# channable/alfred-margaret

Hardware: AMD Instinct MI355X
Metric: GiB/s haystack bytes scanned (match-emitting runLower, 100k-needle automaton) (higher is better)
Workload: dtype u8

## Files before the change

### alfred-margaret_amd/api.py

```python
import ctypes as C
import os

import numpy as np

from . import build as _build

CASE_SENSITIVE = 0
IGNORE_CASE = 1

AM_OK = 0
AM_ERR_INVALID, AM_ERR_NO_DEVICE, AM_ERR_HIP, AM_ERR_OOM, AM_ERR_UNSUPPORTED = -1, -2, -3, -4, -5


class AmError(RuntimeError):
    def __init__(self, code, msg):
        super().__init__("libam error %d: %s" % (code, msg))
        self.code = code


class Slice(C.Structure):
    _fields_ = [("ptr", C.c_void_p), ("off", C.c_size_t), ("len", C.c_size_t)]


MATCH_DTYPE = np.dtype([("end_pos", np.uint64), ("haystack", np.uint32), ("state", np.uint32)])
# ... 947 lines not shown

def sf_unit_chunks(total_bytes, n_cu=0):
    uc = int(libam().am_debug_sf_unit_chunks(int(total_bytes), int(n_cu)))
    if uc == 0:
        raise AmError(AM_ERR_NO_DEVICE, (libam().am_last_error() or b"").decode("utf-8", "replace"))
    return uc


SF_MODES = ("count", "emit", "any", "ids")


def decode_sf_variant(word):
    word = int(word)
    if not word & 1:
        return None
    return {"ic": bool(word & 2), "mode": SF_MODES[(word >> 2) & 3], "ilp": (word >> 4) & 3, "lw": (word >> 16) & 255, "short": bool(word & 64), "dbg": bool(word & 128),
            "light": bool(word & 256), "children": bool(word & 512)}


def sf_last_variant():
    return decode_sf_variant(libam().am_debug_sf_last_variant())


def bounds_report():
    f, l, u = C.c_uint64(0), C.c_uint32(0), C.c_uint32(0)
    check(libam().am_debug_bounds_report(C.byref(f), C.byref(l), C.byref(u)))
    return int(f.value), int(l.value), int(u.value)


def image_version():
    return int(libam().am_image_version())


def lower_code_point(cp):
    return int(libam().am_lower_code_point(cp))


def unlower_code_point(cp):
    buf = (C.c_uint32 * 16)()
    n = libam().am_unlower_code_point(cp, buf, 16)
    return [int(buf[i]) for i in range(n)]


def lower_utf8(text):
    b = _as_bytes(text)
    out = C.create_string_buffer(len(b) * 4 + 4)
# ... 41 lines not shown
```

### alfred-margaret_amd/csrc/am_abi.cpp

```cpp
#include "am_host.h"

#include <condition_variable>
#include <deque>
#include <sys/mman.h>

using namespace am;
using namespace am::dev;
using namespace am::host;

static_assert(sizeof(am_match) == sizeof(Record), "am_match must mirror the device record");
static_assert(offsetof(am_match, end_pos) == offsetof(Record, end_pos) && offsetof(am_match, haystack) == offsetof(Record, haystack) &&
                  offsetof(am_match, state) == offsetof(Record, state), "am_match layout");


static thread_local std::string g_err;
namespace am { int abi_fail(int code, const std::string& msg) { g_err = msg; return code; } }

namespace am {
namespace host {

Runtime g_rt;

int ensure_runtime()
{
// ... 107 lines not shown
    }
    HIP_TRY(hipMemcpyAsync(tl_state.pin_res + off, d_src, n, hipMemcpyDeviceToHost, st));
    items[n_items++] = Item{dst, off, n};
    used = off + n;
    return AM_OK;
}
int am::host::ResultCopies::finish(hipStream_t st)
{
    HIP_TRY(hipStreamSynchronize(st));
    for (int i = 0; i < n_items; i++) std::memcpy(items[i].dst, tl_state.pin_res + items[i].off, items[i].n);
    return AM_OK;
}

namespace {
struct RecordCache {
    struct Block { void* p; size_t cap; };
    std::mutex mu; std::vector<Block> kept;
    void* take(size_t need, size_t* cap_out)
    {
        std::lock_guard<std::mutex> lk(mu);
        size_t best = kept.size();
        for (size_t i = 0; i < kept.size(); i++)
            if (kept[i].cap >= need && kept[i].cap <= 2 * need + (1u << 20) && (best == kept.size() || kept[i].cap < kept[best].cap)) best = i;
        if (best == kept.size()) return nullptr;
        void* r = kept[best].p; *cap_out = kept[best].cap;
        kept.erase(kept.begin() + (std::ptrdiff_t)best);
        return r;
    }
    void trim()
    {
        std::vector<Block> out;
        { std::lock_guard<std::mutex> lk(mu); out.swap(kept); }
        for (const Block& b : out) (void)hipFree(b.p);
    }
    void give(void* q, size_t c)
    {
        std::vector<Block> out;
        {
            std::lock_guard<std::mutex> lk(mu);
            kept.push_back(Block{q, c});
            size_t total = 0;
            for (const Block& b : kept) total += b.cap;
            while (kept.size() > 4 || (kept.size() > 1 && total > ((size_t)16 << 30))) { total -= kept.front().cap; out.push_back(kept.front()); kept.erase(kept.begin()); }
        }
        for (const Block& b : out) (void)hipFree(b.p);
    }
// ... 423 lines not shown
    if (limit == 0) {
        size_t free_b = 0, total_b = 0;
        OnDevice od(dev);
        limit = (od.rc == AM_OK && hipMemGetInfo(&free_b, &total_b) == hipSuccess) ? std::max<size_t>(total_b / 16, (size_t)256 << 20) : (size_t)256 << 20;
        keep[dev].store(limit, std::memory_order_relaxed);
    }
    if (held > limit) { am_batch_destroy(b); b = nullptr; }
}
}

int am::host::upload_batch(const am_slice* hay, size_t n_hay, am_batch* b, bool oneshot) { return upload_slices(hay, n_hay, b, oneshot); }
am_batch* am::host::oneshot_batch(int dev) { return oneshot_get(dev); }
void am::host::oneshot_batch_trim(int dev) { oneshot_trim(dev); }
int am::host::record_array_get(int dev, size_t need, void** p, size_t* cap)
{
    *p = g_record_cache[dev].take(need, cap);
    if (*p) return AM_OK;
    *cap = need + need / 16;
    hipError_t e = hipMalloc(p, *cap);
    if (e != hipSuccess) { *p = nullptr; *cap = 0; return fail(e == hipErrorOutOfMemory ? AM_ERR_OOM : AM_ERR_HIP, std::string("hipMalloc(records): ") + hipGetErrorString(e)); }
    return AM_OK;
}
void am::host::record_array_put(int dev, void* p, size_t cap) { if (p) g_record_cache[dev].give(p, cap); }

extern "C" int am_batch_from_device(const void* d_bytes, const void* d_offsets, size_t n_hay, uint64_t total_bytes, am_batch** out)
{
    if (!out) return fail(AM_ERR_INVALID, "out is null");
    *out = nullptr;
    if (!d_offsets || (total_bytes && !d_bytes)) return fail(AM_ERR_INVALID, "null device pointers");
    int dev = 0;
    AM_TRY(device_of_pointer(total_bytes ? d_bytes : d_offsets, &dev));
    ON_DEVICE(dev);
    if (((uintptr_t)d_bytes & 15) != 0) return fail(AM_ERR_INVALID, "d_bytes must be 16-byte aligned");
    if (n_hay >= 0xFFFFFFFFull) return fail(AM_ERR_INVALID, "too many haystacks");
    uint64_t first = 1, last = 0;
    HIP_TRY(hipMemcpy(&first, d_offsets, 8, hipMemcpyDeviceToHost));
    HIP_TRY(hipMemcpy(&last, (const uint64_t*)d_offsets + n_hay, 8, hipMemcpyDeviceToHost));
    if (first != 0 || last != total_bytes) return fail(AM_ERR_INVALID, "d_offsets[0] must be 0 and d_offsets[n_hay] must equal total_bytes");
    am_batch* b = new am_batch();
    b->dev = dev;
    b->owns = false; b->d_text = const_cast<void*>(d_bytes); b->d_offsets = (uint64_t*)const_cast<void*>(d_offsets);
    b->total = total_bytes; b->n_hay = (uint32_t)n_hay;
    int rc = finish_batch(b);
    if (rc != AM_OK) { am_batch_destroy(b); return rc; }
    *out = b;
    return AM_OK;
// ... 655 lines not shown
```

### alfred-margaret_amd/csrc/am_device.h

```cpp
#pragma once
#include <hip/hip_runtime.h>

#include "am_image.h"

namespace am {
namespace dev {

constexpr int kModeCount = 0;
constexpr int kModeEmit = 1;
constexpr int kModeAny = 2;
constexpr int kModeIds = 3;

struct alignas(16) Record { uint64_t end_pos; uint32_t haystack; uint32_t state; };

struct ScanOut {
    uint32_t* unit_counts;
    const uint64_t* unit_offsets;
    Record* records;
    Record* pool;
    uint32_t* block_next;
    uint32_t* pool_ctrl;
    uint32_t* unit_first;
    uint32_t* unit_slots;
    uint32_t wq_iters;
// ... 2 lines not shown
    uint32_t unit_chunks;
    uint32_t* next_unit;
    uint64_t* hay_counts;
    uint64_t* total_values;
    uint8_t* flags;
    const uint64_t* ids_vals_off; const uint32_t* ids_vals; uint32_t* ids_bits; uint32_t* ids_missing; uint32_t ids_words, ids_n;
    uint32_t two_always;
    uint64_t* dbg;
};

constexpr uint32_t kPoolBlock = 64;
constexpr uint32_t kSfBlockGrant = 32;
inline uint64_t pool_grant_slack(int n_cu, uint64_t n_units, bool two_per_cu)
{
    uint64_t w = (uint64_t)n_cu * (two_per_cu ? 32u : 16u);
    const uint64_t need = (n_units + 15u) / 16u * 16u;
    if (w > need) w = need;
    return w * kSfBlockGrant;
}

hipError_t launch_hidx(const BatchView& b, uint32_t* hidx, uint64_t n_entries, hipStream_t st, uint32_t* z0 = nullptr, uint64_t n0 = 0, uint32_t* z1 = nullptr, uint64_t n1 = 0);
uint64_t sf_chunks(const BatchView& b);
uint32_t sf_unit_chunks(const BatchView& b, int n_cu);
hipError_t launch_permute(const ScanOut& o, const uint64_t* unit_offsets, Record* out, uint64_t n_units, hipStream_t st);
uint64_t ac_units(const AcView& a, const BatchView& b);
size_t sf_lds_bytes(const SfView& s);
hipError_t launch_sf(bool ic, int mode, const SfView& s, const BatchView& b, const ScanOut& o, int n_cu, hipStream_t st);
uint32_t take_sf_last_variant();
hipError_t launch_ac(bool ic, int mode, const AcView& a, const BatchView& b, const ScanOut& o, hipStream_t st);
uint64_t dfa_units(const DfaView& d, const BatchView& b);
bool dfa_usable(const DfaView& d);
struct DfaLaunch {
    int n_cu; uint32_t workgroups, per_cu;
    uint32_t lds_rows, hot_rows, lds_n1, lds_n2;
    uint32_t walk; bool place_wide;
};
DfaLaunch dfa_launch_shape(const DfaView& d, const BatchView& b, int n_cu);
hipError_t launch_dfa(int mode, const DfaView& d, const BatchView& b, const ScanOut& o, const DfaLaunch& s, hipStream_t st);
hipError_t launch_dfa_sample(const DfaView& d, const uint8_t* text, uint64_t total, uint32_t n_samples, uint32_t len, uint32_t* out, hipStream_t st);
bool dfa_tokens_ok(const DfaView& d);
uint64_t dfa_token_superblocks(uint64_t records, uint32_t n_waves , uint64_t n_units);
uint64_t dfa_superblock_bytes();
hipError_t launch_dfa_tokens(const DfaView& d, const BatchView& b, const ScanOut& o, const DfaLaunch& s, hipStream_t st);
hipError_t launch_dfa_place(const DfaView& d, const BatchView& b, const ScanOut& o, uint32_t n_super, const uint64_t* unit_offsets, const DfaLaunch& s, uint32_t n_ref_states, Record* out, hipStream_t st);
hipError_t read_sf_phase_cycles(uint64_t* out5);
hipError_t read_sf_wave_records(uint64_t* out, size_t n_waves);
hipError_t scan_temp_bytes(uint64_t n, size_t* bytes);
hipError_t launch_scan(void* temp, size_t temp_bytes, const uint32_t* counts, uint64_t* offsets, uint64_t n, hipStream_t st);


hipError_t launch_dense(bool ic, bool write, const AcView& a, const BatchView& b, const Record* sparse, const uint64_t* sparse_offsets, uint32_t unit_chunks,
                        uint64_t n_units, uint32_t* unit_totals, const uint64_t* out_offsets, Record* out, hipStream_t st);
hipError_t launch_records_reduce(const Record* recs, uint64_t n, const uint32_t* vlen, uint64_t* hay_counts, uint64_t* total, uint8_t* flags, hipStream_t st);
hipError_t launch_range_bounds(const Record* recs, uint64_t n, uint64_t x0, uint64_t x1, uint64_t* out2, hipStream_t st);
hipError_t launch_range_rebase(Record* recs, uint64_t n, uint64_t add, hipStream_t st);
hipError_t launch_hay_rebase(Record* recs, uint64_t n, uint32_t add, hipStream_t st);
hipError_t launch_spin(uint32_t workgroups, uint32_t threads, uint64_t cycles, uint32_t* out, hipStream_t st);

struct RpPayload { int64_t priority; uint32_t len_bytes; uint32_t len_code_points; uint64_t repl_off; uint32_t repl_len; uint32_t reserved; };
struct RpStateOne { int32_t priority; uint32_t payload; };
constexpr uint32_t kRpWalkList = 0xFFFFFFFFu;
struct RpTables { const uint64_t* vals_off; const uint32_t* vals; const RpPayload* payloads; const uint8_t* repl; int64_t min_priority; const RpStateOne* one; };
struct RpKept { uint64_t src_start, src_len, dst; };
constexpr uint32_t kRpActive = 0, kRpFinished = 1, kRpNothing = 2;
struct RpHay { uint64_t newlen; int64_t best; uint32_t status, nkept, payload, pad; };
struct RpFin { uint64_t off, len; uint32_t orig, status; };
struct RpRoute { uint64_t* len_next; uint64_t* len_fin; uint32_t* tiles; uint32_t* act; uint32_t* fin; };
struct RpRouted { const uint64_t* off_next; const uint64_t* off_fin; const uint64_t* tile_off; const uint64_t* act_idx; const uint64_t* fin_idx; };
constexpr uint64_t kRpTile = 16384;

hipError_t launch_rp_ranges(const Record* recs, uint64_t n_rec, uint64_t* rec_first, const RpRoute& route, uint32_t n_act, hipStream_t st);
// ... 129 lines not shown
```

### alfred-margaret_amd/csrc/am_host.h

```cpp
#pragma once
#include "../../include/am.h"
#include "../../include/am_debug.h"

#include <hip/hip_runtime.h>

#include <algorithm>
#include <atomic>
#include <chrono>
#include <cstdio>
#include <cstdlib>
#include <cstring>
#include <functional>
#include <future>
#include <map>
#include <memory>
#include <mutex>
#include <string>
#include <thread>
#include <vector>

#include "am_config.h"
#include "am_device.h"
#include "am_flatten.h"

// ... 108 lines not shown
    bool has_ref = false;
    std::shared_ptr<const am::LowerTable> lower;
    std::vector<uint8_t> cs_image;
    struct Flat { int rc = 0; std::string err; std::vector<uint8_t> img; };
    std::future<Flat> ic_pending;
    int kernel_pref = 0;
    std::mutex mu;
    am::host::Flavor fl[2];
};

struct am_batch {
    int dev = 0;
    void* d_text = nullptr; uint64_t* d_offsets = nullptr;
    bool owns = false;
    bool hidx_ready = false;
    uint64_t total = 0; uint32_t n_hay = 0;
    std::mutex mu;
    am::host::DevBuf text_buf, offs_buf;
    am::host::DevBuf combo;
    am::host::DevBuf hidx, unit_counts, unit_offsets, scan_tmp, small, hay_counts, flags, unit_first, pool, block_next;
    am::host::DevBuf sparse, dense_counts, dense_offsets, dense_out;
    uint64_t route_image = 0; bool route_dfa = false;
    uint32_t route_ends_per_kib = 0;
};

struct am_matches {
    int dev = 0;
    am::dev::Record* d_records = nullptr; uint64_t n = 0; size_t cap_bytes = 0;
    uint64_t first = 0;
    std::vector<am_match> host; bool fetched = false;
    am_match* big = nullptr; size_t big_cap = 0;
    bool big_pinned = false;
};

struct am_needle_ids {
    const am_automaton* a = nullptr;
    uint32_t n_needles = 0;
    uint64_t n_states = 0, n_values = 0;
    am::host::DevBuf vals_off, vals;
};

namespace am {
namespace host {

struct ResultCopies {
    struct Item { void* dst; size_t off, n; };
    Item items[4]; int n_items = 0; size_t used = 0;
    int add(void* dst, const void* d_src, size_t n, hipStream_t st);
    int finish(hipStream_t st);
};

int prepare(const am_automaton* ca, int case_mode, const Flavor** out);
int finish_batch(am_batch* b);
int run_batch_impl(const am_automaton* a, int case_mode, const am_batch* cb, am_matches** out, bool allow_small);
int scan_needle_ids(const am_automaton* a, int case_mode, am_batch* b, const uint64_t* d_vals_off, const uint32_t* d_vals, uint32_t n_needles,
                    uint32_t* d_bits, uint32_t words, uint32_t* d_missing, uint8_t* flags_out, bool* taken);
int run_records(const am_automaton* a, int case_mode, am_batch* b, const std::function<int(uint64_t, Record**)>& sink_final, uint64_t* n_out, bool have_lock = false);
int run_records_async(const am_automaton* a, int case_mode, am_batch* b, Record* d_out, const uint64_t** n_dev, hipStream_t st);
int upload_batch(const am_slice* hay, size_t n_hay, am_batch* b, bool oneshot);
am_batch* oneshot_batch(int dev);
void oneshot_batch_trim(int dev);
int record_array_get(int dev, size_t need, void** p, size_t* cap);
void record_array_put(int dev, void* p, size_t cap);
struct RecordArray {
    int dev; void* p = nullptr; size_t cap = 0;
    explicit RecordArray(int d) : dev(d) {}
    int ensure(size_t need)
    {
        if (need <= cap) return AM_OK;
        record_array_put(dev, p, cap); p = nullptr; cap = 0;
        return record_array_get(dev, need, &p, &cap);
    }
    ~RecordArray() { record_array_put(dev, p, cap); }
};
inline size_t padded_text(uint64_t total) { return (size_t)((total + 15) & ~15ull) + 16; }
template <class Buf>
auto records_into(Buf& d, uint64_t spare = 0)
{
    return [&d, spare](uint64_t n, Record** ptr) -> int { AM_TRY(d.ensure((n + spare) * sizeof(Record))); *ptr = (Record*)d.p; return AM_OK; };
}
inline constexpr RpRoute kNoRoute{nullptr, nullptr, nullptr, nullptr, nullptr};

}
}
```

### alfred-margaret_amd/csrc/am_kernels.hip

```cpp
#include <hip/hip_runtime.h>

#include <atomic>
#include <cstdlib>
#include <type_traits>

#include "am_bounds.h"
#include "am_config.h"
#include "am_device.h"
#include "am_wave.h"

AM_BOUNDS_TU("am_kernels.hip")

namespace am {
namespace dev {


__global__ void k_hidx(const uint64_t* __restrict__ offsets, uint32_t n_hay, uint64_t total, uint32_t* __restrict__ hidx, uint64_t n_entries,
                       uint32_t* __restrict__ z0, uint64_t n0, uint32_t* __restrict__ z1, uint64_t n1)
{
    const uint64_t k = (uint64_t)blockIdx.x * blockDim.x + threadIdx.x;
    const uint64_t stride = (uint64_t)gridDim.x * blockDim.x;
    for (uint64_t i = k; i < n0; i += stride) z0[i] = 0u;
    for (uint64_t i = k; i < n1; i += stride) z1[i] = 0u;
    if (k >= n_entries) return;
// ... 602 lines not shown
        for (int i = 0; i < 7; i++) atomicAdd(reinterpret_cast<unsigned long long*>(o.dbg + 16 + 2 * 8192 + i), (unsigned long long)dbg_iters[i]);
        atomicAdd(reinterpret_cast<unsigned long long*>(o.dbg + 11), (unsigned long long)n_cand);
        atomicAdd(reinterpret_cast<unsigned long long*>(o.dbg + 12), (unsigned long long)n_probes);
        atomicAdd(reinterpret_cast<unsigned long long*>(o.dbg + 13), (unsigned long long)n_defer);
        atomicAdd(reinterpret_cast<unsigned long long*>(o.dbg + 14), (unsigned long long)n_found);
        atomicMax(reinterpret_cast<unsigned long long*>(o.dbg + 15), (unsigned long long)(__builtin_amdgcn_s_memtime() - t_begin));
        const uint64_t gw = (uint64_t)blockIdx.x * kSfWaves + wave;
        if (gw < 8192) {
            uint32_t hw_id, xcc_id;
            asm volatile("s_getreg_b32 %0, hwreg(HW_REG_HW_ID)" : "=s"(hw_id));
            asm volatile("s_getreg_b32 %0, hwreg(HW_REG_XCC_ID)" : "=s"(xcc_id));
            o.dbg[16 + 2 * gw] = __builtin_amdgcn_s_memtime() - t_begin;
            o.dbg[17 + 2 * gw] = ((uint64_t)xcc_id << 32) | hw_id;
        }
    }

    if (MODE == kModeCount) {
        if (o.hay_counts) flush_count();
        nval = wave_sum_u64(nval);
        if (lane == 0 && nval) atomicAdd(reinterpret_cast<unsigned long long*>(o.total_values), (unsigned long long)nval);
    }
}

__global__ __launch_bounds__(256) void k_permute(ScanOut o, const uint64_t* __restrict__ unit_offsets, Record* __restrict__ out, uint64_t n_units)
{
    const uint64_t u = ((uint64_t)blockIdx.x * blockDim.x + threadIdx.x) >> 6;
    const uint32_t lane = threadIdx.x & 63u;
    if (u >= n_units) return;
    const uint32_t n = o.unit_slots[u];
    uint64_t at = unit_offsets[u];
    uint32_t blk = o.unit_first[u];
    const uint4* pool4 = reinterpret_cast<const uint4*>(o.pool);
    uint4* out4 = reinterpret_cast<uint4*>(out);
    for (uint32_t done = 0; done < n; done += kPoolBlock) {
        if (blk == kNone) break;
        uint4 r = make_uint4(0u, 0u, 0u, kNone);
        if (done + lane < n) r = pool4[(uint64_t)blk * kPoolBlock + lane];
        const uint64_t m = __ballot(r.w != kNone);
        if (r.w != kNone) out4[at + (uint32_t)__popcll(m & ((1ull << lane) - 1ull))] = r;
        at += (uint32_t)__popcll(m);
        blk = o.block_next[blk];
    }
}


hipError_t launch_hidx(const BatchView& b, uint32_t* hidx, uint64_t n_entries, hipStream_t st, uint32_t* z0, uint64_t n0, uint32_t* z1, uint64_t n1)
{
    const uint32_t blocks = (uint32_t)((n_entries + 255) / 256);
    hipLaunchKernelGGL(k_hidx, dim3(blocks), dim3(256), 0, st, b.offsets, b.n_hay, b.total, hidx, n_entries, z0, n0, z1, n1);
    return hipGetLastError();
}

uint64_t sf_chunks(const BatchView& b) { return (b.total + kSfChunk - 1) / kSfChunk; }

uint32_t sf_unit_chunks(const BatchView& b, int n_cu)
{
    const uint64_t n_chunks = sf_chunks(b), waves = (uint64_t)(n_cu > 0 ? n_cu : 1) * kSfWaves;
    const uint64_t per_wave = (n_chunks + waves - 1) / waves;
    const uint64_t k = (per_wave + kSfMaxUnitChunks - 1) / kSfMaxUnitChunks;
    if (k >= 4) return kSfMaxUnitChunks;
    const uint64_t uc = k <= 1 ? per_wave : (n_chunks + waves * k - 1) / (waves * k);
    return (uint32_t)(uc < 1 ? 1 : uc);
}

hipError_t launch_permute(const ScanOut& o, const uint64_t* unit_offsets, Record* out, uint64_t n_units, hipStream_t st)
{
    if (n_units == 0) return hipSuccess;
    const uint64_t blocks = (n_units * 64 + 255) / 256;
    hipLaunchKernelGGL(k_permute, dim3((uint32_t)blocks), dim3(256), 0, st, o, unit_offsets, out, n_units);
    return hipGetLastError();
}
uint64_t ac_units(const AcView& a, const BatchView& b) { return (b.total + a.chunk - 1) / a.chunk; }

static size_t sf_lds_bytes_w(const SfView& s, int waves) { return kSfMaskBytes + ((size_t)4 << s.bloom_log2_words) + (size_t)waves * (kSfStage + kSfQ1 * sizeof(uint16_t) + kSfQ2 * sizeof(uint16_t)); }
static uint32_t sf_wq_cap(const SfView& s, int waves)
{
    const size_t base = sf_lds_bytes_w(s, waves), limit = 160 * 1024;
    if (base >= limit) return 0;
    size_t cap = (limit - base) / ((size_t)waves * 64);
    if (cap > 128) cap = 128;
    return cap >= 64 ? (uint32_t)cap : 0u;
}
size_t sf_lds_bytes(const SfView& s) { return sf_lds_bytes_w(s, kSfWaves); }

constexpr uint32_t kSfVariantValid = 1u, kSfVariantIc = 2u, kSfVariantModeShift = 2, kSfVariantIlpShift = 4, kSfVariantShort = 1u << 6, kSfVariantDbg = 1u << 7,
                   kSfVariantLight = 1u << 8, kSfVariantChildren = 1u << 9, kSfVariantLwShift = 16;
static std::atomic<uint32_t> g_sf_last_variant{0};
uint32_t take_sf_last_variant() { return g_sf_last_variant.exchange(0, std::memory_order_relaxed); }

template <bool IC, int MODE, int ILP, int LW, bool SHORT, bool DBG = false, int NT = kSfThreads, bool CHILDREN = false>
static hipError_t launch_sf_v(const SfView& s, const BatchView& b, const ScanOut& o, int n_cu, hipStream_t st)
{
// ... 97 lines not shown
```

### alfred-margaret_amd/csrc/am_run.cpp

```cpp
#include "am_host.h"

using namespace am;
using namespace am::dev;
using namespace am::host;

namespace {

using AcLauncher = hipError_t (*)(bool ic, int mode, const AcView& a, const BatchView& b, const ScanOut& o, hipStream_t st);
std::atomic<AcLauncher> g_ac_launcher{nullptr};

constexpr uint64_t kDfaMinBytes = 32ull << 20;
constexpr uint64_t kDfaSampleBytes = 32ull << 20;
constexpr uint32_t kDfaEndsPerKiB = 48;

struct Plan {
    const Flavor* f; bool ic; bool use_sf; bool nothing; uint64_t n_units; uint32_t unit_chunks; int n_cu;
    bool use_dfa;
    DfaView dfa;
    DfaLaunch dfa_shape{};
    bool dense;
    AcView ac; SfView sf; BatchView bv;
    am_batch* batch;
    uint32_t* next_unit;
};

int make_plan(const am_automaton* a, int case_mode, am_batch* b, Plan& p, bool allow_dfa = false, bool have_lock = false)
{
    if (!b) return fail(AM_ERR_INVALID, "null batch");
    if (!a) return fail(AM_ERR_INVALID, "null automaton");
    if (a->dev != b->dev) return fail(AM_ERR_INVALID, "automaton and batch live on different devices");
    AM_TRY(prepare(a, case_mode, &p.f));
    p.ic = case_mode == AM_IGNORE_CASE;
// ... 132 lines not shown
    const Plan& p; hipStream_t st; ScanSpace sp;
    ScanOut o{};
    int setup(uint64_t want_blocks)
    {
        am_batch* b = p.batch;
        if (want_blocks >= (1ull << 26)) return fail(AM_ERR_UNSUPPORTED, "too many match records for one call (2^32 record slots); split the batch");
        AM_TRY(b->unit_first.ensure(2 * p.n_units * sizeof(uint32_t)));
        AM_TRY(b->pool.ensure(want_blocks * kPoolBlock * sizeof(Record)));
        AM_TRY(b->block_next.ensure(want_blocks * sizeof(uint32_t)));
        o = ScanOut{};
        o.unit_chunks = p.unit_chunks;
        o.unit_counts = (uint32_t*)b->unit_counts.p;
        o.unit_first = (uint32_t*)b->unit_first.p;
        o.unit_slots = (uint32_t*)b->unit_first.p + p.n_units;
        o.pool = (Record*)b->pool.p;
        o.block_next = (uint32_t*)b->block_next.p;
        o.pool_ctrl = (uint32_t*)b->small.p + 4;
        o.n_blocks = (uint32_t)want_blocks;
        return AM_OK;
    }
    int scan(bool fused_clear, bool jobs_scan)
    {
        am_batch* b = p.batch;
        uint32_t* tail = (uint32_t*)b->unit_counts.p + p.n_units;
        if (fused_clear) AM_TRY(build_hidx_and_clear(p, b, st, b->small.p, 64, tail, sizeof(uint32_t)));
        else {
            HIP_TRY(hipMemsetAsync(b->small.p, 0, 64, st));
            HIP_TRY(hipMemsetAsync(tail, 0, sizeof(uint32_t), st));
            AM_TRY(build_hidx(p, b, st));
        }
        AM_TRY(launch_scan_kernel(p, kModeEmit, o, st));
        Prof pr("scan", st);
        if (jobs_scan && sp.n <= (1u << 16)) {
            ScanJobs jobs{}; jobs.n_jobs = 1;
            jobs.j[0] = ScanJob{(const uint32_t*)b->unit_counts.p, nullptr, (uint64_t*)b->unit_offsets.p, sp.n, nullptr};
            HIP_TRY(launch_scan_jobs(jobs, st));
        } else HIP_TRY(launch_scan(b->scan_tmp.p, sp.tmp_bytes, (const uint32_t*)b->unit_counts.p, (uint64_t*)b->unit_offsets.p, sp.n, st));
        return AM_OK;
    }
    int permute(Record* out) { Prof pr("permute", st); HIP_TRY(launch_permute(o, (const uint64_t*)p.batch->unit_offsets.p, out, p.n_units, st)); return AM_OK; }
};

}

static int reduce_dense(const am_automaton* a, int case_mode, am_batch* b, uint64_t* counts_out, uint64_t* total_out, uint8_t* flags_out)
{
    uint64_t n_rec = 0;
    auto sink = [&](uint64_t n, Record** ptr) -> int { AM_TRY(b->dense_out.ensure(n * sizeof(Record))); *ptr = (Record*)b->dense_out.p; return AM_OK; };
    const Flavor* f = nullptr;
    AM_TRY(prepare(a, case_mode, &f));
    std::lock_guard<std::mutex> lk(b->mu);
    AM_TRY(run_records(a, case_mode, b, sink, &n_rec, true));
    if (n_rec == 0) return AM_OK;
    ON_DEVICE(b->dev);
    hipStream_t st; AM_TRY(get_stream(b->dev, &st));
    AM_TRY(b->small.ensure(64));
    HIP_TRY(hipMemsetAsync(b->small.p, 0, 64, st));
    if (counts_out) { AM_TRY(b->hay_counts.ensure((size_t)b->n_hay * 8)); HIP_TRY(hipMemsetAsync(b->hay_counts.p, 0, (size_t)b->n_hay * 8, st)); }
    if (flags_out) { AM_TRY(b->flags.ensure(b->n_hay)); HIP_TRY(hipMemsetAsync(b->flags.p, 0, b->n_hay, st)); }
    const AcView ac = make_ac_view(f->d_image, f->h);
    HIP_TRY(launch_records_reduce((const Record*)b->dense_out.p, n_rec, ac.vlen, counts_out ? (uint64_t*)b->hay_counts.p : nullptr, (uint64_t*)b->small.p,
                                  flags_out ? (uint8_t*)b->flags.p : nullptr, st));
    uint64_t total = 0;
// ... 68 lines not shown
    *taken = false;
    Plan p; AM_TRY(make_plan(a, case_mode, b, p));
    if (p.nothing || p.dense || !p.use_sf) return AM_OK;
    std::lock_guard<std::mutex> lk(b->mu);
    ON_DEVICE(b->dev);
    hipStream_t st; AM_TRY(get_stream(b->dev, &st));
    AM_TRY(b->flags.ensure(((size_t)b->n_hay + 3) & ~(size_t)3));
    AM_TRY(b->small.ensure(64));
    ScanOut o{};
    o.unit_chunks = p.unit_chunks;
    o.flags = (uint8_t*)b->flags.p;
    o.ids_vals_off = d_vals_off; o.ids_vals = d_vals; o.ids_bits = d_bits; o.ids_missing = d_missing; o.ids_words = words; o.ids_n = n_needles;
    HIP_TRY(hipMemsetAsync(d_bits, 0, (size_t)b->n_hay * words * 4, st));
    HIP_TRY(hipMemsetD32Async((hipDeviceptr_t)d_missing, (int)n_needles, b->n_hay, st));
    AM_TRY(build_hidx_and_clear(p, b, st, b->flags.p, ((size_t)b->n_hay + 3) & ~(size_t)3, b->small.p, 64));
    AM_TRY(launch_scan_kernel(p, kModeIds, o, st));
    ResultCopies rc;
    AM_TRY(rc.add(flags_out, b->flags.p, b->n_hay, st));
    AM_TRY(rc.finish(st));
    *taken = true;
    return AM_OK;
}

int am::host::run_records(const am_automaton* a, int case_mode, am_batch* b, const std::function<int(uint64_t, Record**)>& sink_final, uint64_t* n_out, bool have_lock)
{
    *n_out = 0;
    Plan p; AM_TRY(make_plan(a, case_mode, b, p, true, have_lock));
    if (p.nothing) return AM_OK;
    std::unique_lock<std::mutex> lk(b->mu, std::defer_lock);
    if (!have_lock) lk.lock();
    ON_DEVICE(b->dev);
    hipStream_t st; AM_TRY(get_stream(b->dev, &st));
    uint64_t n_sparse = 0;
    auto sink_sparse = [&](uint64_t n, Record** ptr) -> int { AM_TRY(b->sparse.ensure(n * sizeof(Record))); *ptr = (Record*)b->sparse.p; return AM_OK; };
    const std::function<int(uint64_t, Record**)>& sink = p.dense ? std::function<int(uint64_t, Record**)>(sink_sparse) : sink_final;
    uint64_t* n_scan = p.dense ? &n_sparse : n_out;
    ScanSpace sp; AM_TRY(scan_workspaces(b, p.n_units, &sp));
    const uint64_t n = sp.n; const size_t tmp_bytes = sp.tmp_bytes;
    Record* d_records = nullptr;
    auto body_ac = [&]() -> int {
        ScanOut o{};
        o.unit_counts = (uint32_t*)b->unit_counts.p;
        o.total_values = (uint64_t*)b->small.p;
        HIP_TRY(hipMemsetAsync(b->small.p, 0, 64, st));
        HIP_TRY(hipMemsetAsync((uint32_t*)b->unit_counts.p + p.n_units, 0, sizeof(uint32_t), st));
        AM_TRY(build_hidx(p, b, st));
        AM_TRY(launch_scan_kernel(p, kModeCount, o, st));
// ... 37 lines not shown
            HIP_TRY(hipMemsetAsync(b->small.p, 0, 64, st));
            HIP_TRY(hipMemsetAsync(b->block_next.p, 0, want * sizeof(uint32_t), st));
            HIP_TRY(hipMemsetAsync((uint32_t*)b->unit_counts.p + p.n_units, 0, sizeof(uint32_t), st));
            AM_TRY(build_hidx(p, b, st));
            { Prof pr("dfa", st); HIP_TRY(launch_dfa_tokens(p.dfa, p.bv, o, p.dfa_shape, st)); }
            { Prof pr("scan", st); HIP_TRY(launch_scan(b->scan_tmp.p, tmp_bytes, (const uint32_t*)b->unit_counts.p, (uint64_t*)b->unit_offsets.p, n, st)); }
            uint64_t total = 0; uint32_t ctrl[2] = {0, 0};
            HIP_TRY(hipMemcpyAsync(&total, (uint64_t*)b->unit_offsets.p + p.n_units, 8, hipMemcpyDeviceToHost, st));
            HIP_TRY(hipMemcpyAsync(ctrl, o.pool_ctrl, 8, hipMemcpyDeviceToHost, st));
            HIP_TRY(hipStreamSynchronize(st));
            if (ctrl[1]) { want = dfa_token_superblocks(total, n_waves, p.n_units); continue; }
            *n_scan = total;
            if (total == 0) return AM_OK;
            AM_TRY(sink(total, &d_records));
            { Prof pr("dfa_place", st); HIP_TRY(launch_dfa_place(p.dfa, p.bv, o, ctrl[0] < o.n_blocks ? ctrl[0] : o.n_blocks, (const uint64_t*)b->unit_offsets.p, p.dfa_shape, p.f->h.n_states, d_records, st)); }
            HIP_TRY(hipStreamSynchronize(st));
            return AM_OK;
        }
        return fail(AM_ERR_HIP, "token pool exhausted repeatedly (internal error)");
    };
    auto body_sf = [&]() -> int {
        SfEmit e{p, st, sp};
        uint64_t want_blocks = sf_pool_blocks(p, SfPool::Guess);
        for (int attempt = 0; attempt < 4; attempt++) {
            AM_TRY(e.setup(want_blocks));
            AM_TRY(e.scan(false, false));
            uint64_t total = 0; uint32_t ctrl[4] = {0, 0, 0, 0};
            HIP_TRY(hipMemcpyAsync(&total, (uint64_t*)b->unit_offsets.p + p.n_units, 8, hipMemcpyDeviceToHost, st));
            HIP_TRY(hipMemcpyAsync(ctrl, e.o.pool_ctrl, 16, hipMemcpyDeviceToHost, st));
            HIP_TRY(hipStreamSynchronize(st));
            if (ctrl[2]) return fail(AM_ERR_HIP, kSfWatchdog);
            if (ctrl[1]) { want_blocks = sf_pool_blocks(p, SfPool::Exact, ctrl[0]); continue; }
            *n_scan = total;
            if (total == 0) return AM_OK;
            AM_TRY(sink(total, &d_records));
            AM_TRY(e.permute(d_records));
            HIP_TRY(hipStreamSynchronize(st));
            return AM_OK;
        }
        return fail(AM_ERR_HIP, "record pool overflowed repeatedly (internal error)");
    };
    if (!p.dense) return p.use_sf ? body_sf() : (p.use_dfa && dfa_tokens_ok(p.dfa)) ? body_dfa() : body_ac();
    if (p.f->h.sf_tiers != 0) AM_TRY(body_sf());
    else {
        HIP_TRY(hipMemsetAsync(b->unit_offsets.p, 0, n * sizeof(uint64_t), st));
        AM_TRY(build_hidx(p, b, st));
    }
    AM_TRY(b->sparse.ensure(sizeof(Record)));
    AM_TRY(b->dense_counts.ensure(n * sizeof(uint32_t)));
    AM_TRY(b->dense_offsets.ensure(n * sizeof(uint64_t)));
    HIP_TRY(hipMemsetAsync((uint32_t*)b->dense_counts.p + p.n_units, 0, sizeof(uint32_t), st));
    { Prof pr("dense", st);
      HIP_TRY(launch_dense(p.ic, false, p.ac, p.bv, (const Record*)b->sparse.p, (const uint64_t*)b->unit_offsets.p, p.unit_chunks, p.n_units, (uint32_t*)b->dense_counts.p, nullptr, nullptr, st)); }
    { Prof pr("scan", st); HIP_TRY(launch_scan(b->scan_tmp.p, tmp_bytes, (const uint32_t*)b->dense_counts.p, (uint64_t*)b->dense_offsets.p, n, st)); }
    uint64_t total = 0;
    HIP_TRY(hipMemcpyAsync(&total, (uint64_t*)b->dense_offsets.p + p.n_units, 8, hipMemcpyDeviceToHost, st));
    HIP_TRY(hipStreamSynchronize(st));
    *n_out = total;
    if (total == 0) return AM_OK;
    Record* d_out = nullptr;
    AM_TRY(sink_final(total, &d_out));
    { Prof pr("dense", st);
      HIP_TRY(launch_dense(p.ic, true, p.ac, p.bv, (const Record*)b->sparse.p, (const uint64_t*)b->unit_offsets.p, p.unit_chunks, p.n_units, nullptr, (const uint64_t*)b->dense_offsets.p, d_out, st)); }
    HIP_TRY(hipStreamSynchronize(st));
    return AM_OK;
// ... 16 lines not shown
constexpr uint64_t kSmallRunBytes = 64u << 10;
constexpr uint64_t kSmallRunEager = 256;
static int run_records_small(const am_automaton* a, int case_mode, am_batch* b, am_matches* m, bool* done)
{
    *done = false;
    if (b->total == 0 || b->total > kSmallRunBytes || a->kernel_pref == 3) return AM_OK;
    Plan p; AM_TRY(make_plan(a, case_mode, b, p));
    if (p.nothing || p.dense || !p.use_sf || cfg::get(cfg::kSfPoolBlocks) > 0) return AM_OK;
    std::lock_guard<std::mutex> lk(b->mu);
    ON_DEVICE(b->dev);
    hipStream_t st; AM_TRY(get_stream(b->dev, &st));
    ScanSpace sp; AM_TRY(scan_workspaces(b, p.n_units, &sp));
    SfEmit e{p, st, sp};
    AM_TRY(e.setup(sf_pool_blocks(p, SfPool::Guess)));
    void* d_records = nullptr; size_t cap_bytes = 0;
    AM_TRY(record_array_get(b->dev, (size_t)b->total * sizeof(Record), &d_records, &cap_bytes));
    auto body = [&]() -> int {
        AM_TRY(e.scan(true, false));
        AM_TRY(e.permute((Record*)d_records));
        uint64_t total = 0; uint32_t ctrl[2] = {0, 0};
        const uint64_t eager = b->total < kSmallRunEager ? b->total : kSmallRunEager;
        m->host.resize(eager);
        ResultCopies rc;
        AM_TRY(rc.add(&total, (uint64_t*)b->unit_offsets.p + p.n_units, 8, st));
        AM_TRY(rc.add(ctrl, e.o.pool_ctrl, 8, st));
        AM_TRY(rc.add(m->host.data(), d_records, eager * sizeof(Record), st));
        AM_TRY(rc.finish(st));
        if (ctrl[1]) return AM_OK;
        m->n = total;
        if (total <= eager) { m->host.resize(total); m->fetched = true; }
        else { m->host.clear(); m->fetched = false; }
        *done = true;
        return AM_OK;
    };
    const int rc = body();
    if (rc == AM_OK && *done && m->n) { m->d_records = (Record*)d_records; m->cap_bytes = cap_bytes; }
    else record_array_put(b->dev, d_records, cap_bytes);
    return rc;
}

int am::host::run_batch_impl(const am_automaton* a, int case_mode, const am_batch* cb, am_matches** out, bool allow_small)
{
    if (!out) return fail(AM_ERR_INVALID, "out is null");
    *out = nullptr;
    if (!cb) return fail(AM_ERR_INVALID, "null batch");
    am_matches* m = new am_matches();
    m->dev = cb->dev;
    if (allow_small) {
        bool done = false;
        const int rc = run_records_small(a, case_mode, const_cast<am_batch*>(cb), m, &done);
        if (rc != AM_OK) { am_matches_free(m); return rc; }
        if (done) { *out = m; return AM_OK; }
        m->host.clear(); m->fetched = false; m->n = 0;
    }
    auto sink = [&](uint64_t total, Record** ptr) -> int {
        void* r = nullptr;
        AM_TRY(record_array_get(m->dev, total * sizeof(Record), &r, &m->cap_bytes));
        *ptr = m->d_records = (Record*)r;
        return AM_OK;
    };
    const int rc = run_records(a, case_mode, const_cast<am_batch*>(cb), sink, &m->n);
    if (rc != AM_OK) { am_matches_free(m); return rc; }
    *out = m;
    return AM_OK;
}

extern "C" int am_run_batch(const am_automaton* a, int case_mode, const am_batch* cb, am_matches** out) { return run_batch_impl(a, case_mode, cb, out, true); }

extern "C" int am_debug_set_general_kernel(void* launcher, uint32_t image_version)
{
    if (launcher && image_version != kImageVersion) return fail(AM_ERR_INVALID, "libam_check.so was built against another image version");
    g_ac_launcher.store(reinterpret_cast<AcLauncher>(launcher), std::memory_order_release);
    return AM_OK;
}
```

### alfred-margaret_amd/csrc/am_scan.hip

```cpp
#include <hip/hip_runtime.h>

#include "am_device.h"

namespace am {
namespace dev {

namespace {
constexpr int kScanThreads = 256, kScanPer = 16;
constexpr uint64_t kScanTile = (uint64_t)kScanThreads * kScanPer;

__device__ __forceinline__ uint64_t wave_incl_u64(uint64_t x, uint32_t lane)
{
#pragma unroll
    for (int d = 1; d < 64; d <<= 1) { const uint64_t y = __shfl_up(x, d, 64); if (lane >= (uint32_t)d) x += y; }
    return x;
}

__device__ __forceinline__ uint64_t block_exclusive(uint64_t v, uint64_t* total)
{
    __shared__ uint64_t wsum[kScanThreads / 64];
    const uint32_t lane = threadIdx.x & 63u, w = threadIdx.x >> 6;
    const uint64_t incl = wave_incl_u64(v, lane);
    __syncthreads();
    if (lane == 63u) wsum[w] = incl;
    __syncthreads();
// ... 22 lines not shown
    for (uint64_t i0 = 0; i0 < nt; i0 += kScanThreads) {
        const uint64_t i = i0 + threadIdx.x;
        const uint64_t v = i < nt ? tile_sums[i] : 0;
        uint64_t total;
        const uint64_t ex = block_exclusive(v, &total);
        if (i < nt) tile_sums[i] = carry + ex;
        carry += total;
    }
}

template <class T>
__global__ __launch_bounds__(kScanThreads) void k_scan_apply(const T* __restrict__ in, uint64_t n, const uint64_t* __restrict__ tile_base, uint64_t* __restrict__ out)
{
    const uint64_t i0 = (uint64_t)blockIdx.x * kScanTile + (uint64_t)threadIdx.x * kScanPer;
    uint64_t x[kScanPer], v = 0;
#pragma unroll
    for (int k = 0; k < kScanPer; k++) { x[k] = i0 + k < n ? (uint64_t)in[i0 + k] : 0; v += x[k]; }
    uint64_t total;
    uint64_t run = tile_base[blockIdx.x] + block_exclusive(v, &total);
#pragma unroll
    for (int k = 0; k < kScanPer; k++) { if (i0 + k < n) out[i0 + k] = run; run += x[k]; }
}

template <class T>
hipError_t scan_any(void* temp, size_t temp_bytes, const T* in, uint64_t* out, uint64_t n, hipStream_t st)
{
    if (n == 0) return hipSuccess;
    const uint64_t nt = (n + kScanTile - 1) / kScanTile;
    if (temp_bytes < nt * sizeof(uint64_t) || nt > 0x7FFFFFFFull) return hipErrorInvalidValue;
    uint64_t* tiles = (uint64_t*)temp;
    hipLaunchKernelGGL((k_scan_tile_sums<T>), dim3((uint32_t)nt), dim3(kScanThreads), 0, st, in, n, tiles);
    hipLaunchKernelGGL(k_scan_tiles, dim3(1), dim3(kScanThreads), 0, st, tiles, nt);
    hipLaunchKernelGGL((k_scan_apply<T>), dim3((uint32_t)nt), dim3(kScanThreads), 0, st, in, n, (const uint64_t*)tiles, out);
    return hipGetLastError();
}
}

hipError_t scan_temp_bytes(uint64_t n, size_t* bytes) { *bytes = ((n + kScanTile - 1) / kScanTile + 1) * sizeof(uint64_t); return hipSuccess; }
hipError_t scan64_temp_bytes(uint64_t n, size_t* bytes) { return scan_temp_bytes(n, bytes); }

hipError_t launch_scan(void* temp, size_t temp_bytes, const uint32_t* counts, uint64_t* offsets, uint64_t n, hipStream_t st) { return scan_any<uint32_t>(temp, temp_bytes, counts, offsets, n, st); }
hipError_t launch_scan64(void* temp, size_t temp_bytes, const uint64_t* in, uint64_t* out, uint64_t n, hipStream_t st) { return scan_any<uint64_t>(temp, temp_bytes, in, out, n, st); }

}
}
```

Baseline: 1029.

## Speculatively permute into recycled record buffer and replace three-kernel unit scan

The emit path now borrows the largest cached record array, sized from the previous run's match count, and launches the permute before the first host sync. When the total fits, the second sync and the separate allocate-and-permute round trip are skipped. The three-kernel tile scan is replaced by one kernel in which each block re-sums all earlier counts itself, also writing the total into the small control buffer so a single 32-byte readback replaces two copies. This trades redundant prefix work per block and reliance on match counts staying stable between runs for fewer launches and syncs.

Result: no change. 1031 (median of 6 runs) (+0.2%).

```diff
diff --git a/alfred-margaret_amd/api.py b/alfred-margaret_amd/api.py
--- a/alfred-margaret_amd/api.py
+++ b/alfred-margaret_amd/api.py
@@ -993,6 +993,12 @@
     return decode_sf_variant(libam().am_debug_sf_last_variant())
 
 
+def emit_waits():
+    ms, n = C.c_double(0), C.c_uint64(0)
+    check(libam().am_profile_read(b"wait", C.byref(ms), C.byref(n)))
+    return int(n.value)
+
+
 def bounds_report():
     f, l, u = C.c_uint64(0), C.c_uint32(0), C.c_uint32(0)
     check(libam().am_debug_bounds_report(C.byref(f), C.byref(l), C.byref(u)))
diff --git a/alfred-margaret_amd/csrc/am_abi.cpp b/alfred-margaret_amd/csrc/am_abi.cpp
--- a/alfred-margaret_amd/csrc/am_abi.cpp
+++ b/alfred-margaret_amd/csrc/am_abi.cpp
@@ -153,6 +153,17 @@
         size_t best = kept.size();
         for (size_t i = 0; i < kept.size(); i++)
             if (kept[i].cap >= need && kept[i].cap <= 2 * need + (1u << 20) && (best == kept.size() || kept[i].cap < kept[best].cap)) best = i;
+        if (best == kept.size()) return nullptr;
+        void* r = kept[best].p; *cap_out = kept[best].cap;
+        kept.erase(kept.begin() + (std::ptrdiff_t)best);
+        return r;
+    }
+    void* take_largest(size_t min_bytes, size_t* cap_out)
+    {
+        std::lock_guard<std::mutex> lk(mu);
+        size_t best = kept.size();
+        for (size_t i = 0; i < kept.size(); i++)
+            if (kept[i].cap >= min_bytes && (best == kept.size() || kept[i].cap > kept[best].cap)) best = i;
         if (best == kept.size()) return nullptr;
         void* r = kept[best].p; *cap_out = kept[best].cap;
         kept.erase(kept.begin() + (std::ptrdiff_t)best);
@@ -622,6 +633,12 @@
     return AM_OK;
 }
 void am::host::record_array_put(int dev, void* p, size_t cap) { if (p) g_record_cache[dev].give(p, cap); }
+bool am::host::record_array_guess(int dev, size_t min_bytes, void** p, size_t* cap)
+{
+    *p = g_record_cache[dev].take_largest(min_bytes, cap);
+    if (!*p) *cap = 0;
+    return *p != nullptr;
+}
 
 extern "C" int am_batch_from_device(const void* d_bytes, const void* d_offsets, size_t n_hay, uint64_t total_bytes, am_batch** out)
 {
diff --git a/alfred-margaret_amd/csrc/am_device.h b/alfred-margaret_amd/csrc/am_device.h
--- a/alfred-margaret_amd/csrc/am_device.h
+++ b/alfred-margaret_amd/csrc/am_device.h
@@ -48,7 +48,7 @@
 hipError_t launch_hidx(const BatchView& b, uint32_t* hidx, uint64_t n_entries, hipStream_t st, uint32_t* z0 = nullptr, uint64_t n0 = 0, uint32_t* z1 = nullptr, uint64_t n1 = 0);
 uint64_t sf_chunks(const BatchView& b);
 uint32_t sf_unit_chunks(const BatchView& b, int n_cu);
-hipError_t launch_permute(const ScanOut& o, const uint64_t* unit_offsets, Record* out, uint64_t n_units, hipStream_t st);
+hipError_t launch_permute(const ScanOut& o, const uint64_t* unit_offsets, Record* out, uint64_t n_units, uint64_t cap_records, hipStream_t st);
 uint64_t ac_units(const AcView& a, const BatchView& b);
 size_t sf_lds_bytes(const SfView& s);
 hipError_t launch_sf(bool ic, int mode, const SfView& s, const BatchView& b, const ScanOut& o, int n_cu, hipStream_t st);
@@ -73,6 +73,7 @@
 hipError_t read_sf_wave_records(uint64_t* out, size_t n_waves);
 hipError_t scan_temp_bytes(uint64_t n, size_t* bytes);
 hipError_t launch_scan(void* temp, size_t temp_bytes, const uint32_t* counts, uint64_t* offsets, uint64_t n, hipStream_t st);
+hipError_t launch_scan_units(const uint32_t* counts, uint64_t* offsets, uint64_t* total, uint64_t n, hipStream_t st);
 
 
 hipError_t launch_dense(bool ic, bool write, const AcView& a, const BatchView& b, const Record* sparse, const uint64_t* sparse_offsets, uint32_t unit_chunks,
diff --git a/alfred-margaret_amd/csrc/am_host.h b/alfred-margaret_amd/csrc/am_host.h
--- a/alfred-margaret_amd/csrc/am_host.h
+++ b/alfred-margaret_amd/csrc/am_host.h
@@ -154,6 +154,7 @@
     am::host::DevBuf sparse, dense_counts, dense_offsets, dense_out;
     uint64_t route_image = 0; bool route_dfa = false;
     uint32_t route_ends_per_kib = 0;
+    uint64_t last_run_records = ~0ull;
 };
 
 struct am_matches {
@@ -187,13 +188,24 @@
 int run_batch_impl(const am_automaton* a, int case_mode, const am_batch* cb, am_matches** out, bool allow_small);
 int scan_needle_ids(const am_automaton* a, int case_mode, am_batch* b, const uint64_t* d_vals_off, const uint32_t* d_vals, uint32_t n_needles,
                     uint32_t* d_bits, uint32_t words, uint32_t* d_missing, uint8_t* flags_out, bool* taken);
-int run_records(const am_automaton* a, int case_mode, am_batch* b, const std::function<int(uint64_t, Record**)>& sink_final, uint64_t* n_out, bool have_lock = false);
+constexpr uint64_t kNoLastRun = ~0ull;
+bool record_array_guess(int dev, size_t min_bytes, void** p, size_t* cap);
+void record_array_put(int dev, void* p, size_t cap);
+struct RecordGuess {
+    int dev; void* p = nullptr; size_t cap = 0; bool used = false;
+    explicit RecordGuess(int d) : dev(d) {}
+    RecordGuess(const RecordGuess&) = delete;
+    RecordGuess& operator=(const RecordGuess&) = delete;
+    bool take(size_t min_bytes) { give_back(); return record_array_guess(dev, min_bytes, &p, &cap); }
+    void give_back() { if (p && !used) { record_array_put(dev, p, cap); p = nullptr; cap = 0; } }
+    ~RecordGuess() { give_back(); }
+};
+int run_records(const am_automaton* a, int case_mode, am_batch* b, const std::function<int(uint64_t, Record**)>& sink_final, uint64_t* n_out, bool have_lock = false, RecordGuess* guess = nullptr);
 int run_records_async(const am_automaton* a, int case_mode, am_batch* b, Record* d_out, const uint64_t** n_dev, hipStream_t st);
 int upload_batch(const am_slice* hay, size_t n_hay, am_batch* b, bool oneshot);
 am_batch* oneshot_batch(int dev);
 void oneshot_batch_trim(int dev);
 int record_array_get(int dev, size_t need, void** p, size_t* cap);
-void record_array_put(int dev, void* p, size_t cap);
 struct RecordArray {
     int dev; void* p = nullptr; size_t cap = 0;
     explicit RecordArray(int d) : dev(d) {}
diff --git a/alfred-margaret_amd/csrc/am_kernels.hip b/alfred-margaret_amd/csrc/am_kernels.hip
--- a/alfred-margaret_amd/csrc/am_kernels.hip
+++ b/alfred-margaret_amd/csrc/am_kernels.hip
@@ -648,11 +648,12 @@
     }
 }
 
-__global__ __launch_bounds__(256) void k_permute(ScanOut o, const uint64_t* __restrict__ unit_offsets, Record* __restrict__ out, uint64_t n_units)
+__global__ __launch_bounds__(256) void k_permute(ScanOut o, const uint64_t* __restrict__ unit_offsets, Record* __restrict__ out, uint64_t n_units, uint64_t cap_records)
 {
     const uint64_t u = ((uint64_t)blockIdx.x * blockDim.x + threadIdx.x) >> 6;
     const uint32_t lane = threadIdx.x & 63u;
     if (u >= n_units) return;
+    if (unit_offsets[n_units] > cap_records || o.pool_ctrl[1] != 0u) return;
     const uint32_t n = o.unit_slots[u];
     uint64_t at = unit_offsets[u];
     uint32_t blk = o.unit_first[u];
@@ -689,11 +690,11 @@
     return (uint32_t)(uc < 1 ? 1 : uc);
 }
 
-hipError_t launch_permute(const ScanOut& o, const uint64_t* unit_offsets, Record* out, uint64_t n_units, hipStream_t st)
+hipError_t launch_permute(const ScanOut& o, const uint64_t* unit_offsets, Record* out, uint64_t n_units, uint64_t cap_records, hipStream_t st)
 {
     if (n_units == 0) return hipSuccess;
     const uint64_t blocks = (n_units * 64 + 255) / 256;
-    hipLaunchKernelGGL(k_permute, dim3((uint32_t)blocks), dim3(256), 0, st, o, unit_offsets, out, n_units);
+    hipLaunchKernelGGL(k_permute, dim3((uint32_t)blocks), dim3(256), 0, st, o, unit_offsets, out, n_units, cap_records);
     return hipGetLastError();
 }
 uint64_t ac_units(const AcView& a, const BatchView& b) { return (b.total + a.chunk - 1) / a.chunk; }
diff --git a/alfred-margaret_amd/csrc/am_run.cpp b/alfred-margaret_amd/csrc/am_run.cpp
--- a/alfred-margaret_amd/csrc/am_run.cpp
+++ b/alfred-margaret_amd/csrc/am_run.cpp
@@ -8,6 +8,12 @@
 
 using AcLauncher = hipError_t (*)(bool ic, int mode, const AcView& a, const BatchView& b, const ScanOut& o, hipStream_t st);
 std::atomic<AcLauncher> g_ac_launcher{nullptr};
+void count_emit_wait()
+{
+    if (!g_rt.prof_on.load(std::memory_order_relaxed)) return;
+    std::lock_guard<std::mutex> lk(g_rt.mu);
+    g_rt.prof["wait"].second += 1;
+}
 
 constexpr uint64_t kDfaMinBytes = 32ull << 20;
 constexpr uint64_t kDfaSampleBytes = 32ull << 20;
@@ -186,23 +192,29 @@
     int scan(bool fused_clear, bool jobs_scan)
     {
         am_batch* b = p.batch;
+        const bool jobs = jobs_scan && sp.n <= (1u << 16);
         uint32_t* tail = (uint32_t*)b->unit_counts.p + p.n_units;
-        if (fused_clear) AM_TRY(build_hidx_and_clear(p, b, st, b->small.p, 64, tail, sizeof(uint32_t)));
+        if (fused_clear) AM_TRY(build_hidx_and_clear(p, b, st, b->small.p, 64, tail, jobs ? sizeof(uint32_t) : 0));
         else {
             HIP_TRY(hipMemsetAsync(b->small.p, 0, 64, st));
-            HIP_TRY(hipMemsetAsync(tail, 0, sizeof(uint32_t), st));
+            if (jobs) HIP_TRY(hipMemsetAsync(tail, 0, sizeof(uint32_t), st));
             AM_TRY(build_hidx(p, b, st));
         }
         AM_TRY(launch_scan_kernel(p, kModeEmit, o, st));
         Prof pr("scan", st);
-        if (jobs_scan && sp.n <= (1u << 16)) {
-            ScanJobs jobs{}; jobs.n_jobs = 1;
-            jobs.j[0] = ScanJob{(const uint32_t*)b->unit_counts.p, nullptr, (uint64_t*)b->unit_offsets.p, sp.n, nullptr};
-            HIP_TRY(launch_scan_jobs(jobs, st));
-        } else HIP_TRY(launch_scan(b->scan_tmp.p, sp.tmp_bytes, (const uint32_t*)b->unit_counts.p, (uint64_t*)b->unit_offsets.p, sp.n, st));
-        return AM_OK;
-    }
-    int permute(Record* out) { Prof pr("permute", st); HIP_TRY(launch_permute(o, (const uint64_t*)p.batch->unit_offsets.p, out, p.n_units, st)); return AM_OK; }
+        if (jobs) {
+            ScanJobs jobs1{}; jobs1.n_jobs = 1;
+            jobs1.j[0] = ScanJob{(const uint32_t*)b->unit_counts.p, nullptr, (uint64_t*)b->unit_offsets.p, sp.n, nullptr};
+            HIP_TRY(launch_scan_jobs(jobs1, st));
+        } else HIP_TRY(launch_scan_units((const uint32_t*)b->unit_counts.p, (uint64_t*)b->unit_offsets.p, (uint64_t*)b->small.p, p.n_units, st));
+        return AM_OK;
+    }
+    int permute(Record* out, uint64_t cap_records = ~0ull)
+    {
+        Prof pr("permute", st);
+        HIP_TRY(launch_permute(o, (const uint64_t*)p.batch->unit_offsets.p, out, p.n_units, cap_records, st));
+        return AM_OK;
+    }
 };
 
 }
@@ -317,7 +329,7 @@
     return AM_OK;
 }
 
-int am::host::run_records(const am_automaton* a, int case_mode, am_batch* b, const std::function<int(uint64_t, Record**)>& sink_final, uint64_t* n_out, bool have_lock)
+int am::host::run_records(const am_automaton* a, int case_mode, am_batch* b, const std::function<int(uint64_t, Record**)>& sink_final, uint64_t* n_out, bool have_lock, RecordGuess* guess)
 {
     *n_out = 0;
     Plan p; AM_TRY(make_plan(a, case_mode, b, p, true, have_lock));
@@ -401,25 +413,38 @@
     auto body_sf = [&]() -> int {
         SfEmit e{p, st, sp};
         uint64_t want_blocks = sf_pool_blocks(p, SfPool::Guess);
+        RecordGuess* g = p.dense ? nullptr : guess;
         for (int attempt = 0; attempt < 4; attempt++) {
             AM_TRY(e.setup(want_blocks));
+            if (g && attempt == 0 && b->last_run_records != kNoLastRun) (void)g->take(b->last_run_records * sizeof(Record));
             AM_TRY(e.scan(false, false));
-            uint64_t total = 0; uint32_t ctrl[4] = {0, 0, 0, 0};
-            HIP_TRY(hipMemcpyAsync(&total, (uint64_t*)b->unit_offsets.p + p.n_units, 8, hipMemcpyDeviceToHost, st));
-            HIP_TRY(hipMemcpyAsync(ctrl, e.o.pool_ctrl, 16, hipMemcpyDeviceToHost, st));
+            const uint64_t lent = g && g->p ? g->cap / sizeof(Record) : 0;
+            if (lent) AM_TRY(e.permute((Record*)g->p, lent));
+            uint64_t head[4] = {0, 0, 0, 0};
+            HIP_TRY(hipMemcpyAsync(head, b->small.p, 32, hipMemcpyDeviceToHost, st));
             HIP_TRY(hipStreamSynchronize(st));
-            if (ctrl[2]) return fail(AM_ERR_HIP, kSfWatchdog);
-            if (ctrl[1]) { want_blocks = sf_pool_blocks(p, SfPool::Exact, ctrl[0]); continue; }
+            count_emit_wait();
+            const uint64_t total = head[0];
+            const uint32_t drawn = (uint32_t)head[2], overflow = (uint32_t)(head[2] >> 32), watchdog = (uint32_t)head[3];
+            if (watchdog) return fail(AM_ERR_HIP, kSfWatchdog);
+            if (overflow) { if (g) g->give_back(); want_blocks = sf_pool_blocks(p, SfPool::Exact, drawn); continue; }
             *n_scan = total;
             if (total == 0) return AM_OK;
+            if (lent && total <= lent) { g->used = true; return AM_OK; }
+            if (g) g->give_back();
             AM_TRY(sink(total, &d_records));
             AM_TRY(e.permute(d_records));
             HIP_TRY(hipStreamSynchronize(st));
+            count_emit_wait();
             return AM_OK;
         }
         return fail(AM_ERR_HIP, "record pool overflowed repeatedly (internal error)");
     };
-    if (!p.dense) return p.use_sf ? body_sf() : (p.use_dfa && dfa_tokens_ok(p.dfa)) ? body_dfa() : body_ac();
+    if (!p.dense) {
+        const int rc = p.use_sf ? body_sf() : (p.use_dfa && dfa_tokens_ok(p.dfa)) ? body_dfa() : body_ac();
+        if (rc == AM_OK && guess) b->last_run_records = *n_out;
+        return rc;
+    }
     if (p.f->h.sf_tiers != 0) AM_TRY(body_sf());
     else {
         HIP_TRY(hipMemsetAsync(b->unit_offsets.p, 0, n * sizeof(uint64_t), st));
@@ -482,7 +507,7 @@
         const uint64_t eager = b->total < kSmallRunEager ? b->total : kSmallRunEager;
         m->host.resize(eager);
         ResultCopies rc;
-        AM_TRY(rc.add(&total, (uint64_t*)b->unit_offsets.p + p.n_units, 8, st));
+        AM_TRY(rc.add(&total, b->small.p, 8, st));
         AM_TRY(rc.add(ctrl, e.o.pool_ctrl, 8, st));
         AM_TRY(rc.add(m->host.data(), d_records, eager * sizeof(Record), st));
         AM_TRY(rc.finish(st));
@@ -519,8 +544,10 @@
         *ptr = m->d_records = (Record*)r;
         return AM_OK;
     };
-    const int rc = run_records(a, case_mode, const_cast<am_batch*>(cb), sink, &m->n);
+    RecordGuess guess(m->dev);
+    const int rc = run_records(a, case_mode, const_cast<am_batch*>(cb), sink, &m->n, false, &guess);
     if (rc != AM_OK) { am_matches_free(m); return rc; }
+    if (guess.used) { m->d_records = (Record*)guess.p; m->cap_bytes = guess.cap; guess.p = nullptr; }
     *out = m;
     return AM_OK;
 }
diff --git a/alfred-margaret_amd/csrc/am_scan.hip b/alfred-margaret_amd/csrc/am_scan.hip
--- a/alfred-margaret_amd/csrc/am_scan.hip
+++ b/alfred-margaret_amd/csrc/am_scan.hip
@@ -1,6 +1,7 @@
 #include <hip/hip_runtime.h>
 
 #include "am_device.h"
+#include "am_wave.h"
 
 namespace am {
 namespace dev {
@@ -69,6 +70,57 @@
     for (int k = 0; k < kScanPer; k++) { if (i0 + k < n) out[i0 + k] = run; run += x[k]; }
 }
 
+constexpr int kUnitScanThreads = 1024;
+constexpr uint64_t kUnitScanTile = 4ull * kUnitScanThreads;
+__global__ __launch_bounds__(kUnitScanThreads) void k_scan_units(const uint32_t* __restrict__ counts, uint64_t* __restrict__ offsets, uint64_t* __restrict__ total, uint64_t n)
+{
+    constexpr uint32_t kWaves = kUnitScanThreads / 64;
+    __shared__ uint64_t wave_before[kWaves], wave_tile[kWaves];
+    const uint32_t lane = threadIdx.x & 63u, wave = threadIdx.x >> 6;
+    const uint64_t t0 = (uint64_t)blockIdx.x * kUnitScanTile;
+    uint64_t before = 0;
+#pragma unroll 8
+    for (uint64_t i = (uint64_t)threadIdx.x * 4u; i < t0; i += kUnitScanTile) {
+        const uint4 v = *reinterpret_cast<const uint4*>(counts + i);
+        before += (uint64_t)v.x + v.y + v.z + v.w;
+    }
+    const uint64_t i = t0 + (uint64_t)threadIdx.x * 4u;
+    uint4 v = make_uint4(0u, 0u, 0u, 0u);
+    if (i + 4 <= n) v = *reinterpret_cast<const uint4*>(counts + i);
+    else {
+        if (i < n) v.x = counts[i];
+        if (i + 1 < n) v.y = counts[i + 1];
+        if (i + 2 < n) v.z = counts[i + 2];
+    }
+    const uint32_t mine = v.x + v.y + v.z + v.w;
+    const uint32_t incl = wave_inclusive_sum(mine, lane);
+    before = wave_sum_u64(before);
+    if (lane == 0) wave_before[wave] = before;
+    if (lane == 63u) wave_tile[wave] = incl;
+    __syncthreads();
+    uint64_t base = 0, tile = 0;
+#pragma unroll
+    for (uint32_t k = 0; k < kWaves; k++) {
+        base += wave_before[k];
+        if (k < wave) base += wave_tile[k];
+        tile += wave_tile[k];
+    }
+    const uint64_t at = base + (incl - mine);
+    if (i + 4 <= n) {
+        ulonglong2* o2 = reinterpret_cast<ulonglong2*>(offsets + i);
+        o2[0] = make_ulonglong2(at, at + v.x);
+        o2[1] = make_ulonglong2(at + v.x + v.y, at + v.x + v.y + v.z);
+    } else {
+        if (i < n) offsets[i] = at;
+        if (i + 1 < n) offsets[i + 1] = at + v.x;
+        if (i + 2 < n) offsets[i + 2] = at + v.x + v.y;
+    }
+    if (blockIdx.x == gridDim.x - 1u && threadIdx.x == 0) {
+        offsets[n] = base + tile;
+        *total = base + tile;
+    }
+}
+
 template <class T>
 hipError_t scan_any(void* temp, size_t temp_bytes, const T* in, uint64_t* out, uint64_t n, hipStream_t st)
 {
@@ -87,6 +139,14 @@
 hipError_t scan64_temp_bytes(uint64_t n, size_t* bytes) { return scan_temp_bytes(n, bytes); }
 
 hipError_t launch_scan(void* temp, size_t temp_bytes, const uint32_t* counts, uint64_t* offsets, uint64_t n, hipStream_t st) { return scan_any<uint32_t>(temp, temp_bytes, counts, offsets, n, st); }
+hipError_t launch_scan_units(const uint32_t* counts, uint64_t* offsets, uint64_t* total, uint64_t n, hipStream_t st)
+{
+    if (((uintptr_t)counts & 15u) != 0 || ((uintptr_t)offsets & 31u) != 0) return hipErrorInvalidValue;
+    const uint64_t nt = n ? (n + kUnitScanTile - 1) / kUnitScanTile : 1;
+    if (nt > 0x7FFFFFFFull) return hipErrorInvalidValue;
+    hipLaunchKernelGGL(k_scan_units, dim3((uint32_t)nt), dim3(kUnitScanThreads), 0, st, counts, offsets, total, n);
+    return hipGetLastError();
+}
 hipError_t launch_scan64(void* temp, size_t temp_bytes, const uint64_t* in, uint64_t* out, uint64_t n, hipStream_t st) { return scan_any<uint64_t>(temp, temp_bytes, in, out, n, st); }
 
 }
```
